# oarodriguez/PhD-QMCLib

Hardware: AMD Instinct MI355X
Metric: walker-steps/sec (higher is better)
Workload: dtype f64

## Files before the change

phd_qmclib_amd/csrc/qmc_kernels.h:

```cpp
#pragma once

#include "qmc_device.h"
#include "qmc_sorted64.h"
#include "qmc_sorted128.h"

static constexpr int BLOCK = 256;

static constexpr int BLOCK64 = 64;
template <int G>
struct WalkBlock {
    static constexpr int N = (G == 64) ? BLOCK64 : BLOCK;
};

template <int GPB>
__device__ __forceinline__ long long walker_of_block(unsigned b, int grp)
{
    if (GPB == 1)
        return ((long long)(b >> 7) << 7) + ((b & 7u) << 4) + ((b & 127u) >> 3);
    return (long long)b * GPB + grp;
}

template <int G, int P, bool PAD, bool ZC, bool DMC = false>
struct StepLds {
    static constexpr int NROWS =
        DMC ? SortedCot<false, true, false>::ROWS : 5;
    static constexpr int SORTED =
        (G == 64 && P == 2 && !ZC)   ? NROWS * SortedRows<128>::ROW
        : (G == 64 && P == 1 && !ZC) ? NROWS * SortedRows<64>::ROW
                                     : 0;
    static constexpr int GENERAL = GroupLds<G, P, ZC>::DOUBLES;
    static constexpr int DOUBLES = SORTED > GENERAL ? SORTED : GENERAL;
};

__device__ __forceinline__ long long qmc_uniform(long long v)
{
    const int lo = __builtin_amdgcn_readfirstlane((int)v);
    const int hi = __builtin_amdgcn_readfirstlane((int)(v >> 32));
    return ((long long)hi << 32) | (unsigned int)lo;
}
__device__ __forceinline__ int qmc_opaque(int v)
{
    asm volatile("" : "+v"(v));
    return v;
}
__device__ __forceinline__ double qmc_uniform_f64(double v)
{
    return __longlong_as_double(qmc_uniform(__double_as_longlong(v)));
}
__device__ __forceinline__ double qmc_lane_f64(double v, int k)
{
    const long long b = __double_as_longlong(v);
    const int lo = __builtin_amdgcn_readlane((int)b, k);
    const int hi = __builtin_amdgcn_readlane((int)(b >> 32), k);
    return __longlong_as_double(((long long)hi << 32) | (unsigned int)lo);
}

template <int P>
__device__ __forceinline__ void vmc_accept_lanes(const int (&lab)[P], int n,
                                                 int &src0, int &src1)
{
    src0 = 0;
    src1 = 0;
#pragma unroll
    for (int p = 0; p < P; ++p) {
        const unsigned long long b0 = __ballot(lab[p] == 0);
        const unsigned long long b1 = __ballot(lab[p] == 1);
        if (b0) src0 = ((int)__ffsll((long long)b0) - 1) | (p << 6);
        if (b1) src1 = ((int)__ffsll((long long)b1) - 1) | (p << 6);
    }
    if (n == 1) src1 = src0;
}
template <int P>
__device__ __forceinline__ unsigned int vmc_read_slot(const uint32_t (&wd)[P],
                                                      int src)
{
    unsigned int r = 0u;
#pragma unroll
    for (int p = 0; p < P; ++p)
        if ((src >> 6) == p)
            r = (unsigned)__builtin_amdgcn_readlane((int)wd[p], src & 63);
    return r;
}

static constexpr int LB_P1 = 7;
static constexpr int LB_DMC_P2 = 5;
static constexpr int LB_VMC_P2 = 4;
constexpr int lb_waves(int G, int P, bool ZC, int p2)
{
    return (G == 64 && P == 1) ? LB_P1 : (G == 64 && P == 2 && !ZC) ? p2 : 1;
}


template <int P>
struct DmcSpare {
    static constexpr bool ON = P == 1;
};

static constexpr int RESORT_EVERY = 4;

struct EvalArgs {
    const double *pos;
    double *wf, *energy;
    double *ith, *drift;
    long long nconf;
};

template <int G, int P, bool PAD, bool ZC, typename R = double>
__global__ void __launch_bounds__(WalkBlock<G>::N, lb_waves(G, P, ZC, 1))
evaluate_kernel(const DevModel *__restrict__ mp, EvalArgs a)
{
    const DevModel &m = *mp;
    [[maybe_unused]] constexpr int QMC_SEC_OFF = 0;
    QMC_SECTION("top");
    extern __shared__ double smem[];
    constexpr int GPB = WalkBlock<G>::N / G;
    const int grp = threadIdx.x / G, gl = threadIdx.x % G;
    double *lds = smem + (size_t)grp * GroupLds<G, P, ZC>::DOUBLES;
    const long long w = walker_of_block<GPB>(blockIdx.x, grp);
    const bool active = w < a.nconf;
    if (GPB == 1 && !active) return;
    const long long wr = active ? w : 0;
    const int n = walker_n<G, P, PAD>(m);
    double z[P], z1[P], F[P], ei[P], E, wf;
#pragma unroll
    for (int p = 0; p < P; ++p) {
        int i = lane_particle<G, P, PAD>(m, gl, p);
        z1[p] = (i < n) ? a.pos[wr * n + i] : 0.0;
        z[p] = wrap_box(z1[p], m.L);
    }
    eval_walker<G, P, PAD, true, true, ZC, R>(m, z, z1, gl, lds, F, ei, E, wf);
    if (!active) return;
#pragma unroll
    for (int p = 0; p < P; ++p) {
        int i = lane_particle<G, P, PAD>(m, gl, p);
        if (i < n) {
            if (a.ith) a.ith[w * n + i] = ei[p];
            if (a.drift) a.drift[w * n + i] = F[p];
        }
    }
    if (gl == 0) {
        if (a.wf) a.wf[w] = wf;
        if (a.energy) a.energy[w] = E;
    }
}

struct PrepArgs {
    const double *pos;
    double *drift, *energy;
    long long nconf;
};

template <int G, int P, bool PAD, bool ZC, typename R = double>
__global__ void __launch_bounds__(WalkBlock<G>::N, lb_waves(G, P, ZC, 1))
prepare_kernel(const DevModel *__restrict__ mp, PrepArgs a)
{
    const DevModel &m = *mp;
    [[maybe_unused]] constexpr int QMC_SEC_OFF = 0;
    QMC_SECTION("top");
    extern __shared__ double smem[];
    constexpr int GPB = WalkBlock<G>::N / G;
    const int grp = threadIdx.x / G, gl = threadIdx.x % G;
    double *lds = smem + (size_t)grp * GroupLds<G, P, ZC>::DOUBLES;
    const long long w = walker_of_block<GPB>(blockIdx.x, grp);
    const bool active = w < a.nconf;
    if (GPB == 1 && !active) return;
    const long long wr = active ? w : 0;
    const int n = walker_n<G, P, PAD>(m);
    double z[P], z1[P], F[P], ei[P], E, wf;
#pragma unroll
    for (int p = 0; p < P; ++p) {
        int i = lane_particle<G, P, PAD>(m, gl, p);
        z1[p] = (i < n) ? a.pos[wr * n + i] : 0.0;
        z[p] = wrap_box(z1[p], m.L);
    }
    eval_walker<G, P, PAD, false, false, ZC, R>(m, z, z1, gl, lds, F, ei, E,
                                                wf);
    if (!active) return;
#pragma unroll
    for (int p = 0; p < P; ++p) {
        int i = lane_particle<G, P, PAD>(m, gl, p);
        if (i < n) a.drift[w * n + i] = F[p];
    }
    if (gl == 0) a.energy[w] = E;
}

struct alignas(64) VmcRec {
    double wf;
    double ecarry;
    double sum_e, sum_e2;
    long long n_acc;
    long long spare[3];
};
static_assert(sizeof(VmcRec) == 64, "one record = 8 eight-byte words");
typedef unsigned int VmcRecWords __attribute__((ext_vector_type(16)));
#define QMC_CONST __attribute__((address_space(4)))
__device__ __forceinline__ double vmc_rec_word(const VmcRecWords &r, int k)
{
    return __hiloint2double((int)r[2 * k + 1], (int)r[2 * k]);
}

struct VmcArgs {
    double *pos;
    unsigned short *label;
    VmcRec *rec;
    double *ser_wf, *ser_e;
    unsigned char *ser_stat;
    double *ser_pos;
    const double *tape;
    long long tape_steps;
    long long tape_idx;
    long long W;
    long long y;
    unsigned int nsteps;
    int forced;
    int reset_sums;
    int gaussian;
    unsigned int step;
    unsigned int chain0;
    unsigned long long seed;
    double move_spread;
};

template <int G, int P, bool ZC>
struct VmcFused {
    static constexpr bool ON = G == 64 && !ZC && (P == 1 || P == 2);
};

template <int G, int P, bool PAD, bool ZC, bool LEAN, typename R = double,
          bool STEADY = false>
__global__ void __launch_bounds__(WalkBlock<G>::N, lb_waves(G, P, ZC, LB_VMC_P2))
vmc_step_kernel(const DevModel *__restrict__ mp, VmcArgs a)
{
    static_assert(LEAN || !STEADY, "the steady variant is a LEAN kernel");
    const DevModel &m = *mp;
    [[maybe_unused]] constexpr int QMC_SEC_OFF = 0;
    QMC_SECTION("top");
    extern __shared__ double smem[];
    constexpr int GPB = WalkBlock<G>::N / G;
    const int grp = threadIdx.x / G, gl = threadIdx.x % G;
    static_assert(StepLds<G, P, PAD, ZC>::DOUBLES >= GroupLds<G, P, ZC>::DOUBLES,
                  "eval_walker is the fallback on the same LDS region");
    double *lds = smem + (size_t)grp * StepLds<G, P, PAD, ZC>::DOUBLES;
    const long long w = walker_of_block<GPB>(blockIdx.x, grp);
    const bool active = w < a.W;
    if (GPB == 1 && !active) return;
    const long long wr = active ? w : 0;
    const int n = walker_n<G, P, PAD>(m);
    const unsigned int slot = a.chain0 + (unsigned int)wr;
    const bool forced = !STEADY && a.forced != 0;
    const bool reset_sums = !STEADY && a.reset_sums != 0;

    const long long wl = (G == 64) ? qmc_uniform(wr) : wr;
    double wf_cur, e_cur, se = 0.0, se2 = 0.0;
    long long na = 0;
    if constexpr (G == 64) {
        const VmcRecWords r = *(const QMC_CONST VmcRecWords *)(a.rec + wl);
        wf_cur = vmc_rec_word(r, 0);
        e_cur = vmc_rec_word(r, 1);
        se = vmc_rec_word(r, 2);
        se2 = vmc_rec_word(r, 3);
        na = __double_as_longlong(vmc_rec_word(r, 4));
        if (reset_sums) { se = 0.0; se2 = 0.0; na = 0; }
    } else {
        wf_cur = a.rec[wl].wf;
        e_cur = a.rec[wl].ecarry;
    }

    constexpr bool FUSED = STEADY && VmcFused<G, P, ZC>::ON;
    double zc[P];
    int labc[P];
    int src0 = 0, src1 = 0;
    if constexpr (FUSED) {
#pragma unroll
        for (int p = 0; p < P; ++p) {
            int i = lane_particle<G, P, PAD>(m, gl, p);
            zc[p] = (i < n) ? a.pos[wr * n + i] : 0.0;
            labc[p] = (i < n) ? (int)a.label[wr * n + i] : i;
        }
        vmc_accept_lanes<P>(labc, n, src0, src1);
    }
    bool any_acc = false;
    const unsigned int nst = FUSED ? a.nsteps : 1u;
    bool acc = false;
    [[maybe_unused]] const int gl_top = gl;
    for (unsigned int s = 0; s < nst; ++s) {
    const unsigned int step = a.step + s;
    const int gl = FUSED ? qmc_opaque(gl_top) : gl_top;
    QMC_SECTION("load+philox+wrap");
    double zn[P];
    int labn[P];
    double ua = 1.0;
    unsigned int aw0 = 0u, aw1 = 0u;
    bool has0 = false, has1 = false;
    bool outside = false;
    [[maybe_unused]] uint32_t wacc[P];
#pragma unroll
    for (int p = 0; p < P; ++p) {
        wacc[p] = 0u;
        int i = lane_particle<G, P, PAD>(m, gl, p);
        double zp;
        if constexpr (FUSED) {
            zp = zc[p];
            labn[p] = labc[p];
        } else {
            zp = (i < n) ? a.pos[wr * n + i] : 0.0;
            labn[p] = (i < n) ? (int)a.label[wr * n + i] : i;
        }
        const unsigned li = (unsigned)labn[p];
        double d = 0.0;
        if (!forced && i < n) {
            if (!LEAN && a.tape) {
                double tv = a.tape[(wr * a.tape_steps + a.tape_idx) * (n + 1) + li];
                d = a.gaussian ? a.move_spread * tv
                               : (tv - 0.5) * a.move_spread;
            } else if (!LEAN && a.gaussian) {
                double g0, g1;
                philox_normal2(a.seed, slot, step, li, STREAM_VMC_MOVE, g0,
                               g1);
                d = a.move_spread * g0;
            } else {
                uint32_t w0, w1;
                vmc_move_block(a.seed, slot, step, li, w0, w1);
                d = vmc_move_unit(w0) * a.move_spread;
                if constexpr (FUSED) {
                    wacc[p] = w1;
                } else {
                    if (li == 0u) { aw0 = w1; has0 = true; }
                    if (li == 1u || n == 1) { aw1 = w1; has1 = true; }
                }
            }
        }
        zn[p] = wrap_box(zp + d, m.L);
// ... 395 lines not shown
```

phd_qmclib_amd/csrc/qmc_sorted128.h:

```cpp
#pragma once

#include "qmc_sorted64.h"

template <typename R> struct SlotPair;
template <> struct SlotPair<double> {
    typedef double type __attribute__((ext_vector_type(2)));
};
template <> struct SlotPair<float> {
    typedef float type __attribute__((ext_vector_type(2)));
};
template <typename R>
__device__ __forceinline__ typename SlotPair<R>::type ld_pair(const R *p)
{
    return *(const typename SlotPair<R>::type *)p;
}

__device__ __forceinline__ bool rows_ascending128(const double (&z)[2],
                                                  int nl = 64)
{
    const int lo = __double2loint(z[0]), hi = __double2hiint(z[0]);
    const double up = __hiloint2double(
        __builtin_amdgcn_update_dpp(0, hi, 0x130, 0xf, 0xf, true),
        __builtin_amdgcn_update_dpp(0, lo, 0x130, 0xf, 0xf, true));
    const int lane = threadIdx.x & 63;
    const bool bad = (lane < nl) &
                     ((z[1] < z[0]) | ((lane < nl - 1) & (up < z[1])));
    return __builtin_amdgcn_ballot_w64(bad) == 0ull;
}

__device__ __forceinline__ bool sort_rows128(double (&z)[2], int (&lab)[2], int gl,
                                             int nl = 64)
{
    if (rows_ascending128(z, nl)) return true;
    const int lane = threadIdx.x & 63;
    const int a_up = (lane >= nl - 1 ? lane : lane + 1) << 2;
    const int a_dn = (lane == 0 || lane >= nl ? lane : lane - 1) << 2;
    for (int it = 0; it < 66; ++it) {
        anchor_seam_rows<2>(z, lab, 2 * nl);
        {
            const bool sw = lane < nl && z[1] < z[0];
            const double t = z[0]; const int u = lab[0];
            z[0] = sw ? z[1] : z[0]; lab[0] = sw ? lab[1] : lab[0];
            z[1] = sw ? t : z[1];    lab[1] = sw ? u : lab[1];
        }
        {
            const double up = __hiloint2double(
                __builtin_amdgcn_ds_bpermute(a_up, __double2hiint(z[0])),
                __builtin_amdgcn_ds_bpermute(a_up, __double2loint(z[0])));
            const int lup = __builtin_amdgcn_ds_bpermute(a_up, lab[0]);
            const double dn = __hiloint2double(
                __builtin_amdgcn_ds_bpermute(a_dn, __double2hiint(z[1])),
                __builtin_amdgcn_ds_bpermute(a_dn, __double2loint(z[1])));
            const int ldn = __builtin_amdgcn_ds_bpermute(a_dn, lab[1]);
            const bool t_up = lane < nl - 1 && up < z[1];
            const bool t_dn = lane > 0 && lane < nl && dn > z[0];
            z[1] = t_up ? up : z[1]; lab[1] = t_up ? lup : lab[1];
            z[0] = t_dn ? dn : z[0]; lab[0] = t_dn ? ldn : lab[0];
        }
        if (rows_ascending128(z, nl)) return true;
    }
    return false;
}

__device__ __forceinline__ bool far_partner_ok128(const DevModel &m,
                                                  const double (&z)[2], int gl)
{
    const double zp = __shfl_xor(z[0], 32, 64);
    const double d = (gl < 32) ? (z[1] - zp) + m.L : z[1] - zp;
    return __builtin_amdgcn_ballot_w64(d >= m.L_minus_rm) == 0ull;
}

__device__ __forceinline__ bool far_partner_ok_ring128(const DevModel &m,
                                                       const double (&z)[2],
                                                       int gl, int nl)
{
    const bool live = gl < nl;
    int src = gl - nl / 2;
    const bool wrapped = src < 0;
    if (wrapped) src += nl;
    const double zp = __shfl(z[0], live ? src : gl, 64);
    const double d = wrapped ? (z[1] - zp) + m.L : z[1] - zp;
    return __builtin_amdgcn_ballot_w64(live & (d >= m.L_minus_rm)) == 0ull;
}

template <typename R, bool WF, bool EN, bool REUSE, bool PAD = false>
__device__ __forceinline__ void eval_sorted128(const DevModel &m,
                                               const double (&z)[2], int gl,
                                               double *lds, double (&F)[2],
                                               double &E, double &logwf)
{
    constexpr int G = 64, NS = 128, H = SortedRows<NS>::H,
                  ROW = SortedRows<NS>::ROW;
    constexpr bool COT = SortedCot<WF, EN, REUSE>::ON;
    constexpr bool TAN = SortedCot<WF, EN, REUSE>::TAN;
    typedef SortedCot<WF, EN, REUSE> RowsOf;
    R *lS = (R *)lds, *lC = lS + ROW, *lSU = lS + RowsOf::ROW_SU * ROW,
      *lCU = lS + 3 * ROW, *lZ = lS + RowsOf::ROW_Z * ROW;
    const int n = PAD ? m.n : NS;
    const int nl = n / 2;
    const int K = nl / 2;
    const bool half_last = !PAD || (nl & 1) == 0;
    const int kfull = half_last ? K - 1 : K;
    const bool live = !PAD || gl < nl;
    const unsigned long long live_mask =
        PAD ? __builtin_amdgcn_ballot_w64(live) : ~0ull;
    [[maybe_unused]] constexpr int QMC_SEC_OFF = REUSE ? QMC_NSEC / 2 : 0;
    QMC_SECTION("tables+onebody");
    Own64<R> o[2];
    SortedOneBody ob[2];
    PTab ta[2];
    SortedPub pub[2];
#pragma unroll
    for (int a = 0; a < 2; ++a)
        sorted_particle_setup<R, WF, EN, REUSE, NS, false>(
            m, z[a], 2 * gl + a, (R *)lds, o[a], ob[a], n, ta[a], pub[a]);
#define QMC_S128_ST(row, i, v0, v1)                                           \
        *(typename SlotPair<R>::type *)((row) + (i)) =                        \
            typename SlotPair<R>::type{ (R)(v0), (R)(v1) }
    if (!REUSE && live) {
        const int up = H + 2 * gl, lo = up - n;
        QMC_S128_ST(lS, up, pub[0].s, pub[1].s);
        if (!COT) QMC_S128_ST(lC, up, pub[0].c, pub[1].c);
        QMC_S128_ST(lSU, up, pub[0].su, pub[1].su);
        if (!TAN) QMC_S128_ST(lCU, up, pub[0].cu, pub[1].cu);
        QMC_S128_ST(lZ, up, z[0], z[1]);
        if (lo >= 2) {
            if (COT) {
                QMC_S128_ST(lS, lo, pub[0].s, pub[1].s);
            } else {
                QMC_S128_ST(lS, lo, -pub[0].s, -pub[1].s);
                QMC_S128_ST(lC, lo, -pub[0].c, -pub[1].c);
            }
            QMC_S128_ST(lSU, lo, pub[0].su_lo, pub[1].su_lo);
            if (!TAN) QMC_S128_ST(lCU, lo, pub[0].cu_lo, pub[1].cu_lo);
            QMC_S128_ST(lZ, lo, z[0] - m.L, z[1] - m.L);
        }
    } else if (REUSE && COT && live) {
        const int up = H + 2 * gl, lo = up - n;
        QMC_S128_ST(lS, up, pub[0].s, pub[1].s);
        if (TAN) QMC_S128_ST(lSU, up, pub[0].su, pub[1].su);
        if (lo >= 2) {
            QMC_S128_ST(lS, lo, pub[0].s, pub[1].s);
            if (TAN) QMC_S128_ST(lSU, lo, pub[0].su_lo, pub[1].su_lo);
        }
    }
#undef QMC_S128_ST
    if (!REUSE || COT) {
        __builtin_amdgcn_fence(__ATOMIC_RELEASE, "wavefront");
        __builtin_amdgcn_wave_barrier();
        __builtin_amdgcn_fence(__ATOMIC_ACQUIRE, "wavefront");
    }
    int nb_wave = 0;
    const bool nb_counted = EN && !m.is_free && m.ob_table && m.uniform_barrier;
    if (nb_counted)
        nb_wave = __popcll(__ballot(ob[0].barrier & live)) +
                  __popcll(__ballot(ob[1].barrier & live));
    const R sin_rm = (R)m.sin_rm;
    const R *pS = lS + H + 2 * gl, *pC = (COT ? lZ : lC) + H + 2 * gl,
            *pSU = lSU + H + 2 * gl, *pCU = lCU + H + 2 * gl,
            *pZ = lZ + H + 2 * gl;

    int ring_src = 0;
    if (PAD) ring_src = (live ? (gl == 0 ? nl - 1 : gl - 1) : gl) << 2;
#define QMC_S128_ROR(T)                                                       \
    (PAD ? __hiloint2double(                                                  \
               __builtin_amdgcn_ds_bpermute(ring_src, __double2hiint((double)(T))), \
               __builtin_amdgcn_ds_bpermute(ring_src, __double2loint((double)(T)))) \
         : (double)group_ror1<G>(T))
#define QMC_S128_ALL(cond)                                                    \
    ((__builtin_amdgcn_ballot_w64(cond) | ~live_mask) == ~0ull)
    R Fr[2] = { 0, 0 };
    const double kin1_sum = ob[0].kin1 + ob[1].kin1;
    R T[2] = { 0, 0 };
    R Qall = 0, Qs = 0;
    R PS = 1, PL = 1;
    int eS = 0, eL = 0;
    int ns = 0;

#define QMC_S128_SHORT_XY(oa, bsu, bcu, X, Y)                                 \
    const R Y = TAN ? q_fma((oa).c0, (bsu), (R)1)                             \
                    : (oa).c0 * (bcu) + (oa).s0 * (bsu);                      \
    R X = 0;                                                                  \
    if (EN) X = TAN ? (oa).s0 - (bsu)                                         \
                    : (oa).ks0 * (bcu) - (oa).kc0 * (bsu);
#define QMC_S128_XY(oa, cs, cc, bsu, bcu, X, Y, sh)                           \
    const R Y##_s = COT ? (cs) - (oa).s                         \
                        : (oa).s * (cc) - (oa).c * (cs);   \
    R X = 0;                                                                  \
    if (EN) X = COT ? q_fma((oa).s, (cs), (R)1)               \
                    : (oa).c * (cc) + (oa).s * (cs);       \
    const bool sh = COT ? (cc) > (oa).zt                          \
                        : q_abs(Y##_s) < sin_rm;                              \
     \
    const unsigned long long sh##_m = __builtin_amdgcn_ballot_w64(sh);        \
    R Y = Y##_s;                                                              \
    if (sh) {                                                                 \
        asm volatile("");                                                     \
        const R bsu_ = (bsu);                                                 \
        if (TAN) {                                                            \
            Y = q_fma((oa).c0, bsu_, (R)1);                                   \
            X = (oa).s0 - bsu_;                                               \
        } else {                                                              \
            const R bcu_ = (bcu);                                             \
            Y = (oa).c0 * bcu_ + (oa).s0 * bsu_;                              \
            if (EN) X = (oa).ks0 * bcu_ - (oa).kc0 * bsu_;                    \
        }                                                                     \
    }

    QMC_SECTION("pairs_in_lane");
    {
        const R cs = (R)o[0].s, cc = (R)o[0].c;
        QMC_S128_XY(o[1], cs, cc, pSU[0], pCU[0], X, Y, sh)
        if (WF) { PL *= Y; if (sh) { asm volatile(""); PS *= Y; } }
        if (EN) {
            const R q = pair_div(X, Y);
            Fr[1] += q; Fr[0] -= q;
            Qall = q_fma(q, q, Qall);
            ns += __popcll(sh_m & live_mask);
            if (sh) { asm volatile(""); Qs = q_fma(q, q, Qs); }
        }
    }

    QMC_SECTION("leading_short_steps");
    int k = 1;
    R Pl = 1;
    R Ql = 0;
#define QMC_S128_LEAD(su0, cu0, su1, cu1)                                     \
    {                                                                         \
        QMC_S128_SHORT_XY(o[0], su0, cu0, X00, Y00)                           \
        QMC_S128_SHORT_XY(o[1], su0, cu0, X10, Y10)                           \
        QMC_S128_SHORT_XY(o[0], su1, cu1, X01, Y01)                           \
        QMC_S128_SHORT_XY(o[1], su1, cu1, X11, Y11)                           \
        if (WF) Pl *= (Y00 * Y10) * (Y01 * Y11);                              \
        if (EN) {                                                             \
            const R q00 = pair_div(X00, Y00), q10 = pair_div(X10, Y10);       \
            const R q01 = pair_div(X01, Y01), q11 = pair_div(X11, Y11);       \
            Fr[0] += q00 + q01;                                               \
            Fr[1] += q10 + q11;                                               \
            T[0] -= q00 + q10;                                                \
            T[1] -= q01 + q11;                                                \
            Ql = q_fma(q00, q00, Ql); Ql = q_fma(q10, q10, Ql);               \
            Ql = q_fma(q01, q01, Ql); Ql = q_fma(q11, q11, Ql);               \
            T[0] = (R)QMC_S128_ROR(T[0]);                                     \
            T[1] = (R)QMC_S128_ROR(T[1]);                                     \
        }                                                                     \
    }
    {
        typedef typename SlotPair<R>::type R2;
        R2 asu = ld_pair(pSU - 2), acu = TAN ? asu : ld_pair(pCU - 2);
        R az = pZ[-2];
        R2 bsu = ld_pair(pSU - 4), bcu = TAN ? bsu : ld_pair(pCU - 4);
        R bz = pZ[-4];
        const R zt = o[1].zt;
#pragma clang loop unroll(disable)
        while (k < kfull) {
            if (!QMC_S128_ALL(az > zt)) break;
            QMC_S128_LEAD(asu[0], acu[0], asu[1], acu[1])
            asu = ld_pair(pSU - 2 * (k + 2));
            if (!TAN) acu = ld_pair(pCU - 2 * (k + 2));
            az = pZ[-2 * (k + 2)];
            ++k;
            if (!QMC_S128_ALL(bz > zt)) break;
            QMC_S128_LEAD(bsu[0], bcu[0], bsu[1], bcu[1])
            bsu = ld_pair(pSU - 2 * (k + 2));
            if (!TAN) bcu = ld_pair(pCU - 2 * (k + 2));
            bz = pZ[-2 * (k + 2)];
            ++k;
            if (WF) {
                int e = 0;
                q_fold(Pl, e);
                eS += e; eL += e;
            }
        }
    }
#undef QMC_S128_LEAD
    if (WF) { PS *= Pl; PL *= Pl; }
    if (EN) { Qall += Ql; Qs += Ql; ns += 4 * (k - 1) * nl; }

    QMC_SECTION("rotation_loop_body");
#define QMC_S128_STEP(s0_, c0_, s1_, c1_, kk, LAST)                           \
    {                                                                         \
        const bool mine = live & (!(LAST) || gl < K);                         \
        const typename SlotPair<R>::type su_ = ld_pair(pSU - 2 * (kk)),       \
            cu_ = TAN ? su_ : ld_pair(pCU - 2 * (kk));                        \
        QMC_S128_XY(o[0], s0_, c0_, su_[0], cu_[0], X00, Y00, h00)            \
        QMC_S128_XY(o[1], s0_, c0_, su_[0], cu_[0], X10, Y10, h10)            \
        QMC_S128_XY(o[0], s1_, c1_, su_[1], cu_[1], X01, Y01, h01)            \
        QMC_S128_XY(o[1], s1_, c1_, su_[1], cu_[1], X11, Y11, h11)            \
        if (WF && mine) {                                                     \
            PL *= (Y00 * Y10) * (Y01 * Y11);                                  \
            if (h00) { asm volatile(""); PS *= Y00; }                         \
            if (h10) { asm volatile(""); PS *= Y10; }                         \
            if (h01) { asm volatile(""); PS *= Y01; }                         \
            if (h11) { asm volatile(""); PS *= Y11; }                         \
        }                                                                     \
        if (EN) {                                                             \
            const R q00 = pair_div(X00, Y00), q10 = pair_div(X10, Y10);       \
            const R q01 = pair_div(X01, Y01), q11 = pair_div(X11, Y11);       \
            Fr[0] += q00 + q01;                                               \
            Fr[1] += q10 + q11;                                               \
            if (!(LAST)) {                                                    \
                T[0] -= q00 + q10;                                            \
                T[1] -= q01 + q11;                                            \
                T[0] = (R)QMC_S128_ROR(T[0]);                                 \
                T[1] = (R)QMC_S128_ROR(T[1]);                                 \
            }                                                                 \
            const unsigned long long mine_m =                                 \
                (LAST) ? __builtin_amdgcn_ballot_w64(mine) : live_mask;       \
            ns += __popcll(h00_m & mine_m) + __popcll(h10_m & mine_m) +       \
                  __popcll(h01_m & mine_m) + __popcll(h11_m & mine_m);        \
            if (mine) {                                                       \
                Qall = q_fma(q00, q00, Qall); Qall = q_fma(q10, q10, Qall);   \
                Qall = q_fma(q01, q01, Qall); Qall = q_fma(q11, q11, Qall);   \
                if (h00) { asm volatile(""); Qs = q_fma(q00, q00, Qs); }      \
                if (h10) { asm volatile(""); Qs = q_fma(q10, q10, Qs); }      \
                if (h01) { asm volatile(""); Qs = q_fma(q01, q01, Qs); }      \
                if (h11) { asm volatile(""); Qs = q_fma(q11, q11, Qs); }      \
            }                                                                 \
        }                                                                     \
    }
#define QMC_S128_LONG_XY(oa, cs, cc, X, Y)                                    \
    const R Y = COT ? (cs) - (oa).s : (oa).s * (cc) - (oa).c * (cs);          \
    R X = 0;                                                                  \
    if (EN) X = COT ? q_fma((oa).s, (cs), (R)1)                               \
                    : (oa).c * (cc) + (oa).s * (cs);
#define QMC_S128_LONG_STEP(s0_, c0_, s1_, c1_)                                \
    {                                                                         \
        QMC_S128_LONG_XY(o[0], s0_, c0_, X00, Y00)                            \
        QMC_S128_LONG_XY(o[1], s0_, c0_, X10, Y10)                            \
        QMC_S128_LONG_XY(o[0], s1_, c1_, X01, Y01)                            \
        QMC_S128_LONG_XY(o[1], s1_, c1_, X11, Y11)                            \
        if (WF && live) PL *= (Y00 * Y10) * (Y01 * Y11);                      \
        if (EN) {                                                             \
            const R q00 = pair_div(X00, Y00), q10 = pair_div(X10, Y10);       \
            const R q01 = pair_div(X01, Y01), q11 = pair_div(X11, Y11);       \
            Fr[0] += q00 + q01;                                               \
            Fr[1] += q10 + q11;                                               \
            T[0] -= q00 + q10;                                                \
            T[1] -= q01 + q11;                                                \
            T[0] = (R)QMC_S128_ROR(T[0]);                                     \
            T[1] = (R)QMC_S128_ROR(T[1]);                                     \
            Qall = q_fma(q00, q00, Qall); Qall = q_fma(q10, q10, Qall);       \
            Qall = q_fma(q01, q01, Qall); Qall = q_fma(q11, q11, Qall);       \
        }                                                                     \
    }
    {
        typedef typename SlotPair<R>::type R2;
        R2 as = ld_pair(pS - 2 * k), ac = ld_pair(pC - 2 * k);
        R2 bs = ld_pair(pS - 2 * (k + 1)), bc = ld_pair(pC - 2 * (k + 1));
        const R zt0 = o[0].zt;
#pragma clang loop unroll(disable)
        while (k < kfull) {
            if (__builtin_amdgcn_ballot_w64(live & (pZ[-2 * k + 1] > zt0)) ==
                0ull)
                break;
            QMC_S128_STEP(as[0], ac[0], as[1], ac[1], k, false)
            as = ld_pair(pS - 2 * (k + 2)); ac = ld_pair(pC - 2 * (k + 2));
            QMC_S128_STEP(bs[0], bc[0], bs[1], bc[1], k + 1, false)
            bs = ld_pair(pS - 2 * (k + 3)); bc = ld_pair(pC - 2 * (k + 3));
            k += 2;
            if (WF) {
                q_fold(PS, eS);
                q_fold(PL, eL);
            }
        }
        QMC_SECTION("rotation");
#pragma clang loop unroll(disable)
        while (k < kfull) {
            QMC_S128_LONG_STEP(as[0], ac[0], as[1], ac[1])
            as = ld_pair(pS - 2 * (k + 2)); ac = ld_pair(pC - 2 * (k + 2));
            QMC_S128_LONG_STEP(bs[0], bc[0], bs[1], bc[1])
            bs = ld_pair(pS - 2 * (k + 3)); bc = ld_pair(pC - 2 * (k + 3));
            k += 2;
            if (WF) q_fold(PL, eL);
        }
        if (k <= kfull) {
            QMC_S128_STEP(as[0], ac[0], as[1], ac[1], k, false)
            ++k;
            as = bs; ac = bc;
        }
        QMC_SECTION("rotation_last_step");
        if (half_last) QMC_S128_STEP(as[0], ac[0], as[1], ac[1], k, true)
    }
#undef QMC_S128_STEP
#undef QMC_S128_LONG_STEP
#undef QMC_S128_LONG_XY
#undef QMC_S128_XY
#undef QMC_S128_SHORT_XY
    if (EN) {
        if (PAD) {
            int src = gl + kfull + 1;
            if (src >= nl) src -= nl;
            src = live ? src : gl;
            Fr[0] += __shfl(T[0], src, 64);
            Fr[1] += __shfl(T[1], src, 64);
        } else {
            Fr[0] += __shfl_xor(T[0], G / 2, 64);
            Fr[1] += __shfl_xor(T[1], G / 2, 64);
        }
    }
// ... 39 lines not shown
```

phd_qmclib_amd/csrc/qmc_sorted64.h:

```cpp
#pragma once

#include "qmc_device.h"


template <bool WF, bool EN, bool REUSE>
struct SortedCot {
    static constexpr bool ON = EN && !WF;
    static constexpr bool TAN = ON;
    static constexpr bool COMPACT = TAN && !REUSE;
    static constexpr int ROW_SU = COMPACT ? 1 : 2;
    static constexpr int ROW_Z = COMPACT ? 2 : 4;
    static constexpr int ROWS = COMPACT ? 3 : 5;
};

__device__ __forceinline__ double div_clamped(double x, double y, double tiny)
{
    const double ya = fmax(__builtin_fabs(y), tiny);
    return fast_div(x, __builtin_copysign(ya, y));
}

__device__ __forceinline__ double wave_shr1_f64(double v)
{
    const int lo = __double2loint(v), hi = __double2hiint(v);
    return __hiloint2double(
        __builtin_amdgcn_update_dpp(0, hi, 0x138, 0xf, 0xf, true),
        __builtin_amdgcn_update_dpp(0, lo, 0x138, 0xf, 0xf, true));
}

__device__ __forceinline__ unsigned long long lanes_inverted64(double z,
                                                               int nl = 64)
{
    const bool live = (int)(threadIdx.x & 63) < nl;
    return __builtin_amdgcn_ballot_w64(live & (z < wave_shr1_f64(z)));
}

__device__ __forceinline__ bool lanes_ascending64(double z, int nl = 64)
{
    return lanes_inverted64(z, nl) == 0ull;
}

__device__ __forceinline__ void cmpxchg_pass64(double &z, int &lab, int addr,
                                               int flip)
{
    const int plo = __builtin_amdgcn_ds_bpermute(addr, __double2loint(z));
    const int phi = __builtin_amdgcn_ds_bpermute(addr, __double2hiint(z));
    const int pl = __builtin_amdgcn_ds_bpermute(addr, lab);
    const double zp = __hiloint2double(phi, plo);
    const double d = zp - z;
    const bool take = __hiloint2double(__double2hiint(d) ^ flip,
                                       __double2loint(d)) < 0.0;
    z = take ? zp : z;
    lab = take ? pl : lab;
}

__device__ __forceinline__ bool sort_lanes64(double &z, int &lab, int gl,
                                             int nl = 64)
{
    unsigned long long inv = lanes_inverted64(z, nl);
    if (inv == 0ull) return true;
    const int odd = gl & 1;
    const int pe = gl ^ 1;
    const int addr_even = ((gl >= nl || pe >= nl) ? gl : pe) << 2;
    const int po = odd ? (gl + 1) : (gl - 1);
    const int addr_odd = ((gl >= nl || po < 0 || po >= nl) ? gl : po) << 2;
    const int flip_even = odd << 31;
    const int flip_odd = (odd ^ 1) << 31;
    const unsigned long long ends = 2ull | (1ull << (nl - 1));
    for (int it = 0; it < 140; ++it) {
        if (inv & ends) anchor_seam(z, lab, nl);
        if (inv & 0xAAAAAAAAAAAAAAAAull)
            cmpxchg_pass64(z, lab, addr_even, flip_even);
        if (inv & 0x5555555555555555ull)
            cmpxchg_pass64(z, lab, addr_odd, flip_odd);
        inv = lanes_inverted64(z, nl);
        if (inv == 0ull) return true;
    }
    return false;
}

__device__ __forceinline__ bool far_partner_ok64(const DevModel &m, double z,
                                                 int gl)
{
    const double zp = __shfl_xor(z, 32, 64);
    const double d = (gl < 32) ? (z - zp) + m.L : z - zp;
    return __builtin_amdgcn_ballot_w64(d >= m.L_minus_rm) == 0ull;
}

__device__ __forceinline__ bool far_partner_ok_ring(const DevModel &m, double z,
                                                    int gl, int nl)
{
    const int K = nl / 2;
    const bool live = gl < nl;
    int src = gl - K;
    const bool wrapped = src < 0;
    if (wrapped) src += nl;
    const double zp = __shfl(z, live ? src : gl, 64);
    const double d = wrapped ? (z - zp) + m.L : z - zp;
    return __builtin_amdgcn_ballot_w64(live & (d >= m.L_minus_rm)) == 0ull;
}

template <typename R>
struct Own64 {
    R s, c;
    R s0, c0;
    R ks0, kc0;
    R zt;
};

struct SortedOneBody {
    double ldz = 0.0;
    double kin1 = 0.0;
    double xoff = 0.0;
    double prod1 = 1.0;
    bool barrier = false;
};

template <int NS>
struct SortedRows {
    static constexpr int H = NS / 2 + (NS > 64 ? 2 : 1);
    static constexpr int ROW = NS + H;
    static_assert(NS <= 64 || (H % 2 == 0 && ROW % 2 == 0),
                  "two slots per lane: 16-byte aligned pairs");
};

struct SortedPub {
    double s, c, su, cu, su_lo, cu_lo;
};

template <typename R, bool WF, bool EN, bool REUSE, int NS, bool WRITE = true>
__device__ __forceinline__ void sorted_particle_setup(const DevModel &m, double z,
                                                      int slot, R *tab,
                                                      Own64<R> &o,
                                                      SortedOneBody &ob,
                                                      int n, PTab &ta,
                                                      SortedPub &pub)
{
    constexpr int H = SortedRows<NS>::H, ROW = SortedRows<NS>::ROW;
    typedef SortedCot<WF, EN, REUSE> RowsOf;
    R *lS = tab, *lC = lS + ROW, *lSU = lS + RowsOf::ROW_SU * ROW,
      *lCU = lS + 3 * ROW, *lZ = lS + RowsOf::ROW_Z * ROW;
    TrigRow trow;
    const bool trig_ok = !REUSE && m.trig_table && trig_tab_load(m, z, trow);
    if (!m.is_free && m.ob_table) {
        double lf = 0.0;
        one_body_tab<WF, EN>(m, z, ob.ldz, lf, ob.barrier);
        if (WF) ob.xoff = -lf;
        if (EN) {
            if (m.uniform_barrier)
                ob.kin1 = ob.ldz * ob.ldz;
            else
                ob.kin1 = fma(ob.ldz, ob.ldz,
                              one_body_kin_const(m, z, ob.barrier));
        }
    } else if (!m.is_free) {
        double kp, f1, xo;
        one_body(m, z, ob.ldz, kp, f1, xo);
        if (EN) ob.kin1 = kp;
        if (WF) { ob.prod1 = f1; ob.xoff = xo; }
    }
    __builtin_amdgcn_sched_barrier(0);
    if (REUSE) {
        ta.s = (double)lS[H + slot]; ta.c = (double)lC[H + slot];
        ta.su = (double)lSU[H + slot]; ta.cu = (double)lCU[H + slot];
    } else if (trig_ok) {
        trig_tab_finish(m, trow, ta);
    } else {
        sincos_halfpi(z * m.two_over_L, ta.s, ta.c);
        sincos_halfpi(z * m.k2_2pi, ta.su, ta.cu);
    }
    constexpr bool COT = SortedCot<WF, EN, REUSE>::ON;
    constexpr bool TAN = SortedCot<WF, EN, REUSE>::TAN;
    pub.s = ta.s; pub.c = ta.c; pub.su = ta.su; pub.cu = ta.cu;
    const double s0 = fma(ta.su, m.am_cphi, -(ta.cu * m.am_sphi));
    const double c0 = fma(ta.cu, m.am_cphi, ta.su * m.am_sphi);
    pub.su_lo = fma(ta.su, m.cth, -(ta.cu * m.sth_signed));
    pub.cu_lo = fma(ta.cu, m.cth, ta.su * m.sth_signed);
    if (COT) {
        const double tiny = 1e-70;
        const double d0 = fmax(ta.s, tiny);
        const double d1 = __builtin_copysign(fmax(__builtin_fabs(c0), tiny), c0);
        const double d2 = __builtin_copysign(fmax(__builtin_fabs(ta.cu), tiny),
                                             ta.cu);
        const double d3 = __builtin_copysign(
            fmax(__builtin_fabs(pub.cu_lo), tiny), pub.cu_lo);
        const double p01 = d0 * d1, p23 = d2 * d3, pall = p01 * p23;
        double r = __builtin_amdgcn_rcp(pall);
        r = fma(fma(-pall, r, 1.0), r, r);
        r = fma(fma(-pall, r, 1.0), r, r);
        const double i01 = p23 * r, i23 = p01 * r;
        double cotz = ta.c * (i01 * d1);
        double tA = s0 * (i01 * d0);
        double tB = ta.su * (i23 * d3);
        double tBl = pub.su_lo * (i23 * d2);
        if (sizeof(R) == 4) {
            const double big = 1e18;
            cotz = fmin(fmax(cotz, -big), big); tA = fmin(fmax(tA, -big), big);
            tB = fmin(fmax(tB, -big), big); tBl = fmin(fmax(tBl, -big), big);
        }
        pub.s = cotz;
        pub.c = z;
        o.s0 = (R)(m.m_k2_over_a * tA);
        o.c0 = (R)(tA * m.m_a_over_k2);
        pub.su = m.m_k2_over_a * tB;
        pub.su_lo = m.m_k2_over_a * tBl;
    } else {
        o.s0 = (R)s0; o.c0 = (R)c0;
        if (EN) {
            o.ks0 = (R)(m.m_k2_over_a * s0);
            o.kc0 = (R)(m.m_k2_over_a * c0);
        }
    }
    o.s = (R)pub.s; o.c = (R)pub.c;
    o.zt = (R)(z - m.rm);
    if (WRITE && !REUSE && slot < n) {
        lS[H + slot] = (R)pub.s;
        if (!COT) lC[H + slot] = (R)pub.c;
        lSU[H + slot] = (R)pub.su;
        if (!TAN) lCU[H + slot] = (R)pub.cu;
        lZ[H + slot] = (R)z;
        const int lo = H + slot - n;
        if (lo >= 1) {
            lS[lo] = COT ? (R)pub.s : (R)-pub.s;
            if (!COT) lC[lo] = (R)-pub.c;
            lSU[lo] = (R)pub.su_lo;
            if (!TAN) lCU[lo] = (R)pub.cu_lo;
            lZ[lo] = (R)(z - m.L);
        }
    } else if (WRITE && REUSE && COT && slot < n) {
        lS[H + slot] = (R)pub.s;
        if (TAN) lSU[H + slot] = (R)pub.su;
        const int lo = H + slot - n;
        if (lo >= 1) {
            lS[lo] = (R)pub.s;
            if (TAN) lSU[lo] = (R)pub.su_lo;
        }
    }
}

template <typename R, bool WF, bool EN, bool REUSE, bool PAD = false>
__device__ __forceinline__ void eval_sorted64(const DevModel &m, double z, int gl,
                                              double *lds, double &F, double &E,
                                              double &logwf)
{
    constexpr int G = 64, H = SortedRows<G>::H, ROW = SortedRows<G>::ROW;
    constexpr bool COT = SortedCot<WF, EN, REUSE>::ON;
    constexpr bool TAN = SortedCot<WF, EN, REUSE>::TAN;
    typedef SortedCot<WF, EN, REUSE> RowsOf;
    R *lS = (R *)lds, *lC = lS + ROW, *lSU = lS + RowsOf::ROW_SU * ROW,
      *lCU = lS + 3 * ROW, *lZ = lS + RowsOf::ROW_Z * ROW;
    const int nl = PAD ? m.n : G;
    const int K = nl / 2;
    const bool half_last = !PAD || (nl & 1) == 0;
    const int kfull = half_last ? K - 1 : K;
    const bool live = !PAD || gl < nl;
    const unsigned long long live_mask =
        PAD ? __builtin_amdgcn_ballot_w64(live) : ~0ull;
    [[maybe_unused]] constexpr int QMC_SEC_OFF = REUSE ? QMC_NSEC / 2 : 0;
    QMC_SECTION("tables+onebody");
    Own64<R> o;
    SortedOneBody ob;
    PTab ta_own;
    SortedPub pub_own;
    sorted_particle_setup<R, WF, EN, REUSE, G>(m, z, gl, (R *)lds, o, ob, nl,
                                               ta_own, pub_own);
    if (!REUSE || COT) {
        __builtin_amdgcn_fence(__ATOMIC_RELEASE, "wavefront");
        __builtin_amdgcn_wave_barrier();
        __builtin_amdgcn_fence(__ATOMIC_ACQUIRE, "wavefront");
    }
    const double ldz = ob.ldz, kin1 = ob.kin1, xoff = ob.xoff,
                 prod1 = ob.prod1;
    int nb_wave = 0;
    const bool nb_counted = EN && !m.is_free && m.ob_table && m.uniform_barrier;
    if (nb_counted) nb_wave = __popcll(__ballot(ob.barrier & live));
    const R sin_rm = (R)m.sin_rm;
    const R *pS = lS + H + gl, *pC = (COT ? lZ : lC) + H + gl,
            *pSU = lSU + H + gl, *pCU = lCU + H + gl, *pZ = lZ + H + gl;
    int ring_src = 0;
    if (PAD) ring_src = (live ? (gl == 0 ? nl - 1 : gl - 1) : gl) << 2;
#define QMC_S64_ROR(T)                                                        \
    (PAD ? __hiloint2double(                                                  \
               __builtin_amdgcn_ds_bpermute(ring_src, __double2hiint((double)(T))), \
               __builtin_amdgcn_ds_bpermute(ring_src, __double2loint((double)(T)))) \
         : (double)group_ror1<G>(T))

    R Fr = 0;
    R T = 0;
    R Qall = 0, Qs = 0;
    R PS = 1, PL = 1;
    int eS = 0, eL = 0;
    int ns = 0;
    int k = 1;

    QMC_SECTION("leading_short_steps");
#define QMC_S64_LEAD_XY(bsu, bcu, X, Y)                                       \
    const R Y = TAN ? q_fma(o.c0, (bsu), (R)1)                \
                    : o.c0 * (bcu) + o.s0 * (bsu);   \
    R X = 0;                                                                  \
    if (EN) X = TAN ? o.s0 - (bsu)                              \
                    : o.ks0 * (bcu) - o.kc0 * (bsu);                          \
    if (WF) PS *= Y;
#define QMC_S64_ADD_Q(q, kk)                                                  \
    {                                                                         \
        Fr += (q);                                                            \
        T -= (q);                                                             \
        T = (R)QMC_S64_ROR(T);                                                \
    }
#define QMC_S64_ALL(cond)                                                     \
    ((__builtin_amdgcn_ballot_w64(cond) | ~live_mask) == ~0ull)
    {
        R asu = pSU[-1], acu = TAN ? (R)0 : pCU[-1],
          az = pZ[-1];
        R bsu = pSU[-2], bcu = TAN ? (R)0 : pCU[-2],
          bz = pZ[-2];
#pragma clang loop unroll(disable)
        while (k < kfull) {
            if (!QMC_S64_ALL(bz > o.zt)) break;
            QMC_S64_LEAD_XY(asu, acu, Xa, Ya)
            asu = pSU[-(k + 2)];
            if (!TAN) acu = pCU[-(k + 2)];
            az = pZ[-(k + 2)];
            QMC_S64_LEAD_XY(bsu, bcu, Xb, Yb)
            bsu = pSU[-(k + 3)];
            if (!TAN) bcu = pCU[-(k + 3)];
            bz = pZ[-(k + 3)];
            k += 2;
            if (EN) {
                const R qa = pair_div(Xa, Ya), qb = pair_div(Xb, Yb);
                QMC_S64_ADD_Q(qa, k - 2)
                QMC_S64_ADD_Q(qb, k - 1)
                Qs = q_fma(qa, qa, Qs);
                Qs = q_fma(qb, qb, Qs);
            }
            if (WF && sizeof(R) == 4 && (k & 7) == 1) q_fold(PS, eS);
        }
    }
#undef QMC_S64_LEAD_XY
    if (WF) { PL = PS; eL = eS; }
    if (EN) { Qall = Qs; ns = (k - 1) * nl; }

    QMC_SECTION("rotation_loop_body");
#define QMC_S64_XY(cs, cc, kk, LAST, X, Y, sh, mine)                          \
    const R Y##_s = COT ? (cs) - o.s                            \
                        : o.s * (cc) - o.c * (cs);    \
    R X = 0;                                                                  \
    if (EN) X = COT ? q_fma(o.s, (cs), (R)1)                  \
                    : o.c * (cc) + o.s * (cs);             \
    const bool mine = live & (!(LAST) || gl < K);                             \
    const bool sh = COT ? (cc) > o.zt                             \
                        : q_abs(Y##_s) < sin_rm;                              \
         \
    const unsigned long long sh##_m =                                         \
        __builtin_amdgcn_ballot_w64(sh & mine);                               \
    if (EN) ns += __popcll(sh##_m);                                           \
    R Y = Y##_s;                                                              \
    if (sh) {                                                                 \
        asm volatile("");                        \
        const R bsu_ = pSU[-(kk)];                                            \
        if (TAN) {                                                            \
            Y = q_fma(o.c0, bsu_, (R)1);                                      \
            X = o.s0 - bsu_;                                                  \
        } else {                                                              \
            const R bcu_ = pCU[-(kk)];                                        \
            Y = o.c0 * bcu_ + o.s0 * bsu_;                                    \
            if (EN) X = o.ks0 * bcu_ - o.kc0 * bsu_;                          \
        }                                                                     \
        if (WF && mine) PS *= Y;                                              \
    }                                                                         \
    if (WF && mine) PL *= Y;
#define QMC_S64_TALLY(q, sh, mine)                                            \
    if (mine) {                                                               \
        Qall = q_fma(q, q, Qall);                                             \
        if (sh) {                                                             \
            asm volatile("");                                                 \
            Qs = q_fma(q, q, Qs);                                             \
        }                                                                     \
    }
    R as_ = pS[-k], ac_ = pC[-k];
    R bs_ = pS[-(k + 1)], bc_ = pC[-(k + 1)];
#pragma clang loop unroll(disable)
    while (k < kfull) {
        QMC_S64_XY(as_, ac_, k, false, Xa, Ya, sha, minea)
        as_ = pS[-(k + 2)]; ac_ = pC[-(k + 2)];
        QMC_S64_XY(bs_, bc_, k + 1, false, Xb, Yb, shb, mineb)
        bs_ = pS[-(k + 3)]; bc_ = pC[-(k + 3)];
        k += 2;
        if (EN) {
            const R qa = pair_div(Xa, Ya), qb = pair_div(Xb, Yb);
            QMC_S64_ADD_Q(qa, k - 2)
            QMC_S64_ADD_Q(qb, k - 1)
            QMC_S64_TALLY(qa, sha, minea)
            QMC_S64_TALLY(qb, shb, mineb)
        }
        if (WF && sizeof(R) == 4) {
            q_fold(PS, eS);
            q_fold(PL, eL);
        }
        if (shb_m == 0ull) break;
    }
    QMC_SECTION("rotation");
#define QMC_S64_LONG(cs, cc)                                                  \
    {                                                                         \
        const R Y = COT ? (cs) - o.s : o.s * (cc) - o.c * (cs);               \
        if (WF && live) PL *= Y;                                              \
        if (EN) {                                                             \
            const R X = COT ? q_fma(o.s, (cs), (R)1)                          \
                            : o.c * (cc) + o.s * (cs);                        \
            const R q = pair_div(X, Y);                                       \
            QMC_S64_ADD_Q(q, k)                                               \
            if (live) Qall = q_fma(q, q, Qall);                               \
        }                                                                     \
        ++k;                                                                  \
    }
#pragma clang loop unroll(disable)
    while (k < kfull) {
        QMC_S64_LONG(pS[-k], pC[-k])
        QMC_S64_LONG(pS[-k], pC[-k])
        if (WF && sizeof(R) == 4) q_fold(PL, eL);
    }
    as_ = pS[-k]; ac_ = pC[-k];
    bs_ = pS[-(k + 1)]; bc_ = pC[-(k + 1)];
#undef QMC_S64_LONG
    if (k <= kfull) {
        QMC_S64_XY(as_, ac_, k, false, Xa, Ya, sha, minea)
        if (EN) {
            const R q = pair_div(Xa, Ya);
            QMC_S64_ADD_Q(q, k)
            QMC_S64_TALLY(q, sha, minea)
        }
        ++k;
        as_ = bs_; ac_ = bc_;
    }
    QMC_SECTION("rotation_last_step");
    if (half_last) {
        QMC_S64_XY(as_, ac_, k, true, Xl, Yl, shl, minel)
        if (EN) {
            const R q = pair_div(Xl, Yl);
            Fr += q;
            QMC_S64_TALLY(q, shl, minel)
        }
    }
#undef QMC_S64_XY
#undef QMC_S64_TALLY
#undef QMC_S64_ADD_Q
#undef QMC_S64_ALL
    if (EN) {
        if (PAD) {
            int src = gl + kfull + 1;
            if (src >= nl) src -= nl;
            Fr += __shfl(T, live ? src : gl, 64);
        } else {
            Fr += __shfl_xor(T, G / 2, 64);
        }
    }
#undef QMC_S64_ROR

    QMC_SECTION("energy+logwf");
    double e_lane = 0.0, e_consts = 0.0;
    if (EN) {
        F = fma(m.a_long, (double)Fr, ldz);
        const double Qall_d = (double)Qall, Qs_d = (double)Qs;
        const double pk = (Qs_d + (Qall_d - Qs_d) * m.inv_beta) * m.a_long_sq;
        e_lane = fma(2.0, pk, kin1) - F * F;
        if (PAD && !live) e_lane = 0.0;
        if (nb_counted)
            e_consts += (double)(nl - nb_wave) * m.e0 +
                        (double)nb_wave * (m.v_barrier - m.v0_minus_e0);
        const int nlong = nl * (nl - 1) / 2 - ns;
        e_consts += 2.0 * (m.k2sq * (double)ns + m.b_long * (double)nlong);
    }
    double lw = 0.0;
    if (WF) {
        const double LN2 = 0.693147180559945309417;
        const double PS_d = (double)PS, PL_d = (double)PL;
        if (sizeof(R) == 8 && !m.is_free && m.ob_table) {
            const bool odd = gl & 1;
            double own = odd ? PS_d : PL_d, give = odd ? PL_d : PS_d;
            if (PAD && !live) { own = 1.0; give = 1.0; }
            const double got = __hiloint2double(
                __builtin_amdgcn_update_dpp(0, __double2hiint(give), 0xB1, 0xf,
                                            0xf, false),
                __builtin_amdgcn_update_dpp(0, __double2loint(give), 0xB1, 0xf,
                                            0xf, false));
            int bh = __double2hiint(m.beta), bl = __double2loint(m.beta);
            int oh = __double2hiint(m.one_minus_beta),
                ol = __double2loint(m.one_minus_beta);
            asm volatile("" : "+s"(bh), "+s"(bl), "+s"(oh), "+s"(ol));
            lw = __hiloint2double(odd ? oh : bh, odd ? ol : bl) *
                 log_pos(own * got);
            if (PAD && gl >= ((nl + 1) & ~1)) lw = 0.0;
            if (!PAD || live) lw -= xoff;
        } else if (!m.is_free && m.ob_table) {
            const double lSv = log_pos(PS_d);
            lw = fma(m.beta, log_pos(PL_d) - lSv, lSv);
        } else {
            lw = log_pos(prod1 * PS_d) +
                 m.beta * log_pos(fast_div(PL_d, PS_d));
        }
        const bool merged = sizeof(R) == 8 && !m.is_free && m.ob_table;
        if (sizeof(R) == 4)
            lw += LN2 * ((double)eS + m.beta * (double)(eL - eS));
        if (!merged) {
            lw -= xoff;
            if (PAD && !live) lw = 0.0;
        }
    }
    if (WF && EN) {
        E = wave_sum_mfma(e_lane);
        logwf = wave_sum_mfma(lw);
        E += e_consts;
    } else if (EN) {
        E = wave_sum_mfma(e_lane) + e_consts;
    } else {
        logwf = wave_sum_mfma(lw);
    }
}
```

Before: 767.7 million.

## Stage pairwise force terms in LDS instead of rotating accumulator across lanes

Replaces the per-step lane rotation of the Newton-third-law accumulator (DPP/bpermute ror) in the 64-slot sorted evaluator with LDS stores into a staging row, indexed by partner offset, followed by a wave-local read and subtraction. The final cross-lane shuffle to fold the rotated accumulator back is dropped. LDS row layout is reshuffled (new ROW_CU, ROW_Z, staging region) and the LDS budget grows to cover the staging entries. It adds two stores, a load and wave barriers with fences per step, which may cost more than the single rotate it replaces.

```diff
diff --git a/phd_qmclib_amd/csrc/qmc_kernels.h b/phd_qmclib_amd/csrc/qmc_kernels.h
--- a/phd_qmclib_amd/csrc/qmc_kernels.h
+++ b/phd_qmclib_amd/csrc/qmc_kernels.h
@@ -26,8 +26,10 @@
         DMC ? SortedCot<false, true, false>::ROWS : 5;
     static constexpr int SORTED =
         (G == 64 && P == 2 && !ZC)   ? NROWS * SortedRows<128>::ROW
-        : (G == 64 && P == 1 && !ZC) ? NROWS * SortedRows<64>::ROW
+        : (G == 64 && P == 1 && !ZC) ? SortedStage<DMC>::END
                                      : 0;
+    static_assert(!DMC || SortedCot<false, true, false>::COMPACT,
+                  "the staging row follows the three rows");
     static constexpr int GENERAL = GroupLds<G, P, ZC>::DOUBLES;
     static constexpr int DOUBLES = SORTED > GENERAL ? SORTED : GENERAL;
 };
diff --git a/phd_qmclib_amd/csrc/qmc_sorted128.h b/phd_qmclib_amd/csrc/qmc_sorted128.h
--- a/phd_qmclib_amd/csrc/qmc_sorted128.h
+++ b/phd_qmclib_amd/csrc/qmc_sorted128.h
@@ -95,7 +95,7 @@
     constexpr bool TAN = SortedCot<WF, EN, REUSE>::TAN;
     typedef SortedCot<WF, EN, REUSE> RowsOf;
     R *lS = (R *)lds, *lC = lS + ROW, *lSU = lS + RowsOf::ROW_SU * ROW,
-      *lCU = lS + 3 * ROW, *lZ = lS + RowsOf::ROW_Z * ROW;
+      *lCU = lS + RowsOf::ROW_CU * ROW, *lZ = lS + RowsOf::ROW_Z * ROW;
     const int n = PAD ? m.n : NS;
     const int nl = n / 2;
     const int K = nl / 2;
diff --git a/phd_qmclib_amd/csrc/qmc_sorted64.h b/phd_qmclib_amd/csrc/qmc_sorted64.h
--- a/phd_qmclib_amd/csrc/qmc_sorted64.h
+++ b/phd_qmclib_amd/csrc/qmc_sorted64.h
@@ -9,7 +9,8 @@
     static constexpr bool TAN = ON;
     static constexpr bool COMPACT = TAN && !REUSE;
     static constexpr int ROW_SU = COMPACT ? 1 : 2;
-    static constexpr int ROW_Z = COMPACT ? 2 : 4;
+    static constexpr int ROW_Z = COMPACT ? 2 : 3;
+    static constexpr int ROW_CU = 4;
     static constexpr int ROWS = COMPACT ? 3 : 5;
 };
 
@@ -123,6 +124,15 @@
                   "two slots per lane: 16-byte aligned pairs");
 };
 
+template <bool COMPACT>
+struct SortedStage {
+    static constexpr int LO = 31;
+    static constexpr int ENTRIES = LO + 2 * 64 - 1;
+    static constexpr int START =
+        (COMPACT ? 3 : 5) * SortedRows<64>::ROW - (COMPACT ? 0 : LO);
+    static constexpr int END = START + ENTRIES;
+};
+
 struct SortedPub {
     double s, c, su, cu, su_lo, cu_lo;
 };
@@ -138,7 +148,7 @@
     constexpr int H = SortedRows<NS>::H, ROW = SortedRows<NS>::ROW;
     typedef SortedCot<WF, EN, REUSE> RowsOf;
     R *lS = tab, *lC = lS + ROW, *lSU = lS + RowsOf::ROW_SU * ROW,
-      *lCU = lS + 3 * ROW, *lZ = lS + RowsOf::ROW_Z * ROW;
+      *lCU = lS + RowsOf::ROW_CU * ROW, *lZ = lS + RowsOf::ROW_Z * ROW;
     TrigRow trow;
     const bool trig_ok = !REUSE && m.trig_table && trig_tab_load(m, z, trow);
     if (!m.is_free && m.ob_table) {
@@ -247,7 +257,7 @@
     constexpr bool TAN = SortedCot<WF, EN, REUSE>::TAN;
     typedef SortedCot<WF, EN, REUSE> RowsOf;
     R *lS = (R *)lds, *lC = lS + ROW, *lSU = lS + RowsOf::ROW_SU * ROW,
-      *lCU = lS + 3 * ROW, *lZ = lS + RowsOf::ROW_Z * ROW;
+      *lCU = lS + RowsOf::ROW_CU * ROW, *lZ = lS + RowsOf::ROW_Z * ROW;
     const int nl = PAD ? m.n : G;
     const int K = nl / 2;
     const bool half_last = !PAD || (nl & 1) == 0;
@@ -276,16 +286,12 @@
     const R sin_rm = (R)m.sin_rm;
     const R *pS = lS + H + gl, *pC = (COT ? lZ : lC) + H + gl,
             *pSU = lSU + H + gl, *pCU = lCU + H + gl, *pZ = lZ + H + gl;
-    int ring_src = 0;
-    if (PAD) ring_src = (live ? (gl == 0 ? nl - 1 : gl - 1) : gl) << 2;
-#define QMC_S64_ROR(T)                                                        \
-    (PAD ? __hiloint2double(                                                  \
-               __builtin_amdgcn_ds_bpermute(ring_src, __double2hiint((double)(T))), \
-               __builtin_amdgcn_ds_bpermute(ring_src, __double2loint((double)(T)))) \
-         : (double)group_ror1<G>(T))
+    static_assert(!EN || TAN, "the energy passes stage in the unused row");
+    typedef SortedStage<RowsOf::COMPACT> Stage;
+    R *const pT = lS + Stage::START + Stage::LO + gl;
 
     R Fr = 0;
-    R T = 0;
+    R Tp = 0;
     R Qall = 0, Qs = 0;
     R PS = 1, PL = 1;
     int eS = 0, eL = 0;
@@ -300,11 +306,22 @@
     if (EN) X = TAN ? o.s0 - (bsu)                              \
                     : o.ks0 * (bcu) - o.kc0 * (bsu);                          \
     if (WF) PS *= Y;
+#define QMC_S64_STAGE_SYNC                                                    \
+    {                                                                         \
+        __builtin_amdgcn_fence(__ATOMIC_RELEASE, "wavefront");                \
+        __builtin_amdgcn_wave_barrier();                                      \
+        __builtin_amdgcn_fence(__ATOMIC_ACQUIRE, "wavefront");                \
+    }
 #define QMC_S64_ADD_Q(q, kk)                                                  \
     {                                                                         \
         Fr += (q);                                                            \
-        T -= (q);                                                             \
-        T = (R)QMC_S64_ROR(T);                                                \
+         \
+        if (live) pT[-(kk)] = (q);                                            \
+        __builtin_amdgcn_wave_barrier();                                      \
+        if (live) pT[nl - (kk)] = (q);                                        \
+        QMC_S64_STAGE_SYNC                                                    \
+        Tp -= pT[0];                                                          \
+        QMC_S64_STAGE_SYNC                                                    \
     }
 #define QMC_S64_ALL(cond)                                                     \
     ((__builtin_amdgcn_ballot_w64(cond) | ~live_mask) == ~0ull)
@@ -443,17 +460,9 @@
 #undef QMC_S64_XY
 #undef QMC_S64_TALLY
 #undef QMC_S64_ADD_Q
+#undef QMC_S64_STAGE_SYNC
 #undef QMC_S64_ALL
-    if (EN) {
-        if (PAD) {
-            int src = gl + kfull + 1;
-            if (src >= nl) src -= nl;
-            Fr += __shfl(T, live ? src : gl, 64);
-        } else {
-            Fr += __shfl_xor(T, G / 2, 64);
-        }
-    }
-#undef QMC_S64_ROR
+    if (EN) Fr += live ? Tp : (R)0;
 
     QMC_SECTION("energy+logwf");
     double e_lane = 0.0, e_consts = 0.0;
```

Result: slower. 713.8 million (-7.0%).
